# ajzhai/PEANUT

Measured on AMD Instinct MI355X. Metric: maps/sec for 480x480x(4+N_cat) prediction fwd, batch 32, higher is better.
Workload: dtype f32; 1 GPU; 480x480, 14-channel (4+10) partial maps -> 6-class prediction forward (PSPNet R50-V1c-D8), batch 32 per GPU, seeded random-init weights; survey_config=2, global_batch=32, parallelism=dp1 (map shards, no data-path collective)

## Files before the change

### peanut_amd/csrc/conv_pw_ares.hip

```cpp
#include <stdlib.h>

#include "common.h"
#include "conv_common.h"

namespace peanut {

namespace {

typedef const __attribute__((address_space(1))) void* gptr_t;
typedef __attribute__((address_space(3))) void* lptr_t;

__device__ __forceinline__ float load_uncounted(const float* ptr) {
  float v;
  asm volatile("global_load_dword %0, %1, off" : "=v"(v) : "v"(ptr) : "memory");
  return v;
}
template <int CH>
__device__ __forceinline__ void wait_uncounted(const float (&r)[CH], float a, float b) {
  static_assert(CH == 4 || CH == 8, "chunk of 4 or 8 values");
  __builtin_amdgcn_sched_barrier(0);
  if constexpr (CH == 4)
    asm volatile("s_waitcnt vmcnt(0)" ::"v"(r[0]), "v"(r[1]), "v"(r[2]), "v"(r[3]), "v"(a), "v"(b) : "memory");
  else
    asm volatile("s_waitcnt vmcnt(0)" ::"v"(r[0]), "v"(r[1]), "v"(r[2]), "v"(r[3]), "v"(r[4]), "v"(r[5]), "v"(r[6]), "v"(r[7]), "v"(a), "v"(b)
                 : "memory");
  __builtin_amdgcn_sched_barrier(0);
}

template <int NK, bool FLUSH>
__global__ __launch_bounds__(512) void conv_pw_ares_kernel(const ConvKParams p) {
  constexpr int BK = 32, K = NK * BK, TILE = 128 * BK;
  constexpr int CH = 32 / NK;
  static_assert(NK == 4 || NK == 8, "K = 128 or 256");
  __shared__ __attribute__((aligned(1024))) float smem[(NK + 2) * TILE];
  float* const bst = smem + NK * TILE;

  const int tid = threadIdx.x, lane = tid & 63;
  const int wave = __builtin_amdgcn_readfirstlane(tid >> 6);
  const int lr = lane >> 3, lp = lane & 7;
  const int wm = wave >> 2, wn = wave & 3;
  const int li = lane & 31, hi = lane >> 5;
  const bool late = p.phase_shift && wave >= 4;

  const int G = gridDim.x, bid = blockIdx.x;
  const int lw = (bid & 7) * (G >> 3) + (bid >> 3);
  const int NT = p.ntiles;
  const long long U = (long long)p.mtiles * NT;
  const int u0 = (int)(U * lw / G), u1 = (int)(U * (lw + 1) / G);
  if (u0 >= u1) return;

  const int pbn = p.ares_pbn;
  unsigned a_off[2], b_off[2];
#pragma unroll
  for (int j = 0; j < 2; ++j) {
    const int r = (wave * 2 + j) * 8 + lr;
    const int c = lp ^ ((r >> 1) & 7);
    a_off[j] = r * K + c * 4;
    b_off[j] = (r / pbn) * (NK * pbn * BK) + (r % pbn) * BK + c * 4;
  }
  auto dma_a = [&](int mt, int s) {
    const float* base = p.x + (size_t)mt * (128 * K) + s * BK;
#pragma unroll
    for (int j = 0; j < 2; ++j)
      __builtin_amdgcn_global_load_lds((gptr_t)(base + a_off[j]), (lptr_t)(smem + s * TILE + (wave * 2 + j) * 256), 16, 0, 0);
  };
  auto dma_b = [&](int mt, int nt, int kt, int stage) {
    const float* base = p.w + (p.mt_per_group ? (size_t)(mt / p.mt_per_group) * p.w_group_stride : 0) + (size_t)nt * (128 * K) + kt * (pbn * BK);
#pragma unroll
    for (int j = 0; j < 2; ++j)
      __builtin_amdgcn_global_load_lds((gptr_t)(base + b_off[j]), (lptr_t)(bst + stage * TILE + (wave * 2 + j) * 256), 16, 0, 0);
  };

  const int swz = (li >> 1) & 7;
  int sw[4];
#pragma unroll
  for (int ks = 0; ks < 4; ++ks) sw[ks] = ((ks * 2 + hi) ^ swz) * 4;
  const int a_row = (wm * 64 + li) * BK;
  const int b_row = (wn * 32 + li) * BK;

  f32x16 acc[2], acc2[2], prev[2];
#pragma unroll
  for (int t = 0; t < 2; ++t)
#pragma unroll
    for (int r = 0; r < 16; ++r) { acc[t][r] = 0.f; acc2[t][r] = 0.f; prev[t][r] = 0.f; }

  const size_t lane_el = (size_t)(wm * 64 + 4 * hi) * p.cout + wn * 32 + li;
  const bool has_res = p.res != nullptr;
  const size_t rstride = has_res ? (size_t)p.cout : 0;
  const size_t ostride = (size_t)p.cout;
  const float* res_run = has_res ? p.res + lane_el : p.zeros;
  float* out_run = p.y + lane_el;
  const float* prev_sc = p.scale + wn * 32 + li;
  const float* prev_sh = p.shift + wn * 32 + li;
  bool prev_valid = false;
  float scv = 1.f, shv = 0.f;
  const float alpha = p.alpha;
  const bool relu = p.relu != 0;

#define ARES_CHUNK_LOADS(kt)                                                              \
  float resv[CH];                                                                         \
  if ((kt) == 0) {                                                                        \
    scv = load_uncounted(prev_sc);                                                        \
    shv = load_uncounted(prev_sh);                                                        \
  }                                                                                       \
  _Pragma("unroll") for (int i = 0; i < CH; ++i)                                          \
    resv[i] = load_uncounted(res_run + (size_t)(8 * (i >> 2) + (i & 3)) * rstride);       \
  res_run += (size_t)(2 * CH) * rstride;
#define ARES_CHUNK_FINISH(kt)                                                             \
  if (prev_valid) {                                                   \
    _Pragma("unroll") for (int i = 0; i < CH; ++i) {                                      \
      const int idx = (kt) * CH + i;                                                      \
      float v = prev[idx >> 4][idx & 15] * (scv * alpha) + shv;                           \
      v += resv[i];                                                                       \
      if (relu) v = relu_keep_nan(v);                                                     \
      out_run[(size_t)(8 * (i >> 2) + (i & 3)) * ostride] = v;                            \
    }                                                                                     \
  }                                                                                       \
  out_run += (size_t)(2 * CH) * ostride;

  {
    const int mt = u0 / NT, nt = u0 - mt * NT;
#pragma unroll
    for (int s = 0; s < NK; ++s) dma_a(mt, s);
    dma_b(mt, nt, 0, 0);
    asm volatile("s_waitcnt vmcnt(0)" ::: "memory");
    __builtin_amdgcn_s_barrier();
    asm volatile("" ::: "memory");
  }

  int stage = 0;
  for (int u = u0; u < u1; ++u) {
    const int mt = u / NT, nt = u - mt * NT;
    const bool nxt = u + 1 < u1;
    const int mt_n = nxt ? (u + 1) / NT : mt;
    const int nt_n = nxt ? (u + 1) - mt_n * NT : 0;
    const bool refill_next = nxt && mt_n != mt;

    static_for<NK>([&](auto kc) {
      constexpr int kt = decltype(kc)::value;
      const float* const cur_b = bst + stage * TILE;
      const float* const cur_a = smem + kt * TILE;
      const bool more = (kt + 1 < NK) || nxt;
      ARES_CHUNK_LOADS(kt)
      auto request = [&]() {
        if (more) {
          if (kt + 1 < NK) dma_b(mt, nt, kt + 1, stage ^ 1);
          else dma_b(mt_n, nt_n, 0, stage ^ 1);
        }
      };
      if (!late) request();
      __builtin_amdgcn_sched_barrier(0);
      f32x4 af[4][2], bf[4];
#pragma unroll
      for (int j = 0; j < 4; ++j) {
        af[j][0] = *reinterpret_cast<const f32x4*>(cur_a + a_row + sw[j]);
        af[j][1] = *reinterpret_cast<const f32x4*>(cur_a + a_row + 32 * BK + sw[j]);
        bf[j] = *reinterpret_cast<const f32x4*>(cur_b + b_row + sw[j]);
      }
#pragma unroll
      for (int j = 0; j < 2; ++j)
#pragma unroll
        for (int kk = 0; kk < 4; ++kk)
#pragma unroll
          for (int t = 0; t < 2; ++t) acc[t] = __builtin_amdgcn_mfma_f32_32x32x2f32(af[j][t][kk], bf[j][kk], acc[t], 0, 0, 0);
      __builtin_amdgcn_sched_barrier(0);
      if (late) request();
      __builtin_amdgcn_sched_barrier(0);
#pragma unroll
      for (int j = 2; j < 4; ++j)
#pragma unroll
        for (int kk = 0; kk < 4; ++kk)
#pragma unroll
          for (int t = 0; t < 2; ++t) acc[t] = __builtin_amdgcn_mfma_f32_32x32x2f32(af[j][t][kk], bf[j][kk], acc[t], 0, 0, 0);
      if (FLUSH && (kt & 1)) {
#pragma unroll
        for (int t = 0; t < 2; ++t) {
          acc2[t] += acc[t];
#pragma unroll
          for (int r = 0; r < 16; ++r) acc[t][r] = 0.f;
        }
      }
      wait_uncounted<CH>(resv, scv, shv);
      ARES_CHUNK_FINISH(kt)
      if (kt >= 1) { if (refill_next) dma_a(mt_n, kt - 1); }
      asm volatile("s_waitcnt lgkmcnt(0)" ::: "memory");
      __builtin_amdgcn_s_barrier();
      asm volatile("" ::: "memory");
      stage ^= 1;
    });

#pragma unroll
    for (int t = 0; t < 2; ++t) {
      prev[t] = FLUSH ? acc2[t] : acc[t];
#pragma unroll
      for (int r = 0; r < 16; ++r) { acc[t][r] = 0.f; acc2[t][r] = 0.f; }
    }
    {
      const size_t unit_el = (size_t)mt * 128 * p.cout + (size_t)nt * 128 + lane_el;
      res_run = has_res ? p.res + unit_el : p.zeros;
      out_run = p.y + unit_el;
      const int ss_off = (p.mt_per_group && p.ss_group_stride) ? (mt / p.mt_per_group) * p.ss_group_stride : 0;
      prev_sc = p.scale + ss_off + nt * 128 + wn * 32 + li;
      prev_sh = p.shift + ss_off + nt * 128 + wn * 32 + li;
      prev_valid = true;
    }
    if (refill_next) dma_a(mt_n, NK - 1);
  }

  static_for<NK>([&](auto kc) {
    constexpr int kt = decltype(kc)::value;
    ARES_CHUNK_LOADS(kt)
    wait_uncounted<CH>(resv, scv, shv);
    ARES_CHUNK_FINISH(kt)
  });
#undef ARES_CHUNK_LOADS
#undef ARES_CHUNK_FINISH
}

template <int NK, bool FLUSH>
int launch_ares_t(ConvKParams p, hipStream_t stream) {
  int dev = 0, cus = 0;
  if (hipGetDevice(&dev) != hipSuccess || hipDeviceGetAttribute(&cus, hipDeviceAttributeMultiprocessorCount, dev) != hipSuccess || cus < 8)
    return fail(-3, "conv_pw_ares: no current device");
  const long long U = (long long)p.mtiles * p.ntiles;
  long long G = U < cus ? U : cus;
  G -= G % 8;
  if (G < 8) return fail(-2, "conv_pw_ares: launch too small");
  hipLaunchKernelGGL((conv_pw_ares_kernel<NK, FLUSH>), dim3((unsigned)G), dim3(512), 0, stream, p);
  hipError_t e = hipGetLastError();
  if (e != hipSuccess) return fail(-3, std::string("conv_pw_ares launch: ") + hipGetErrorString(e));
  return 0;
}

}

bool conv_pw_uses_ares(int cin, int cout, long long M, int stride, bool two_source, int flush_ktiles, int bn_tile) {
  const bool on = opt(OPT_PW_ARES) != 0;
  const long long min_units = opt(OPT_PW_ARES_MINUNITS);
  if (!on || two_source || (cin != 128 && cin != 256) || stride != 1 || M % 128 != 0 || cout % 128 != 0) return false;
  if (bn_tile != 64 && bn_tile != 128) return false;
  if (flush_ktiles != 0 && flush_ktiles != 2) return false;
  return (M / 128) * (cout / 128) >= min_units;
}

int launch_conv_pw_ares(const ConvKParams& p0, int bn_tile, hipStream_t stream) {
  ConvKParams p = p0;
  p.phase_shift = opt(OPT_PW256_PHASE) != 0;
  p.ares_pbn = bn_tile;
  p.mtiles = p.M / 128;
  p.ntiles = p.cout / 128;
  note_kernel("conv_pw_ares_128x128");
  const bool flush = p.flush == 2;
  if (p.c1 == 256) return flush ? launch_ares_t<8, true>(p, stream) : launch_ares_t<8, false>(p, stream);
  return flush ? launch_ares_t<4, true>(p, stream) : launch_ares_t<4, false>(p, stream);
}

}
```

### peanut_amd/csrc/options.h

```cpp
#pragma once
#include <stdlib.h>
#include <string.h>

#include <string>

namespace peanut {

enum OptionId {
  OPT_PW_GLDS, OPT_PW256_MINK, OPT_PW256_MINTILES, OPT_PW256_PHASE, OPT_PW256_SKIP_PAD, OPT_PW256W_MINK, OPT_PW256W_MINTILES, OPT_PW256P_MINK, OPT_PW256P_MINTILES, OPT_PW256P_FLUSH, OPT_PW256P_ORDER, OPT_PW256P_STREAMK, OPT_PW256WP_MINK, OPT_PW256WP_MINTILES, OPT_PW256WP_NPRE, OPT_PW256WP_STAGGER, OPT_PW_ARES, OPT_PW_SKINNY,
  OPT_PW_ARES_MINUNITS, OPT_PATCH_MINTILES, OPT_STEM_NCHW, OPT_BN64_MAXK, OPT_PW_BN64_MAXK, OPT_PW64_MAXTILES, OPT_FP32_BK, OPT_NCHUNK, OPT_RES_PREFETCH, OPT_SPLIT_MODEL,
  OPT_RS_CONV, OPT_RS_BN64_MAXK, OPT_RS256_MINK, OPT_RS256_MINTILES, OPT_RS64_MAXK, OPT_RS64_MAXTILES,
  OPT_WINO_M, OPT_WINO_HEAD_M, OPT_WINO6_MAXDIL, OPT_WINO5_MINDIL, OPT_WINO_FLUSH_CH, OPT_WINO_MIN_CIN, OPT_WINO_NARROW_MINPIX, OPT_WINO_SMALL_MAXWG, OPT_DEFER_SPLITK,
  OPT_PPM_OVERLAP, OPT_PPM_GROUPED, OPT_PPM_TERM_ROWS, OPT_PPM_GROUP_ROWS, OPT_RCNN_WINO_M, OPT_RCNN_STEM_S2D, OPT_RCNN_RPN_FUSED, OPT_RCNN_FPN_OVERLAP, OPT_RCNN_RANK_SORT, OPT_RCNN_TOPK_SLICE, OPT_RCNN_NMS_LEVELS, OPT_FMM_LOCAL32, OPT_FMM_MAX_PASSES, OPT_FMM_BLOCKED, OPT_FMM_INNER,
  OPT_COUNT
};

struct OptionInfo {
  const char* key;
  long long def;
  bool upload_time;
  const char* help;
};

inline const OptionInfo* option_table() {
  static const OptionInfo t[OPT_COUNT] = {
      {"pw_glds", 1, false, "fp32 1x1 convs / grouped GEMMs on the LDS-DMA kernels of conv_pw.hip (0: conv_igemm)"},
      {"pw256_mink", 1024, false, "fewest input channels for the 256 x 128 three-stage kernel"},
      {"pw256_mintiles", 256, false, "fewest 256 x 128 tiles for that kernel"},
      {"pw256_phase", 1, false, "the two waves of a SIMD request their LDS-DMA pieces half an iteration apart"},
      {"pw256_skip_pad", 1, false, "256 x 128 kernel, grouped GEMMs: waves whose rows are all group padding issue no MFMAs (0: compute the zero rows)"},
      {"pw256w_mink", 768, false, "fewest input channels for the 256 x 256 two-stage kernel (0: off)"},
      {"pw256w_mintiles", 1536, false, "fewest 256 x 256 tiles for that kernel"},
      {"pw256p_mink", 512, false, "fewest input channels for the persistent 256 x 128 kernel (conv_pw256p.hip; 0: off)"},
      {"pw256p_mintiles", 512, false, "fewest 256 x 128 tiles for that kernel"},
      {"pw256p_flush", 512, false, "most input channels of a Winograd position GEMM (two-level accumulation) that runs on the persistent kernel (0: none)"},
      {"pw256p_order", 1, false, "persistent 256 x 128 kernel: 1 = the workgroups of an XCD walk its run of tiles side by side (neighbours share operand panels in L2), 0 = one contiguous run per workgroup"},
      {"pw256p_streamk", 1, false, "persistent 256 x 128 kernel: the tail tiles' k-tiles as one stream in equal runs per workgroup (0: every tail tile cut into the same number of parts)"},
      {"pw256wp_mink", 512, false, "fewest input channels for the persistent 256 x 256 kernel (conv_pw256wp.hip; 0: off)"},
      {"pw256wp_mintiles", 768, false, "fewest 256 x 256 tiles for that kernel"},
      {"pw256wp_npre", 0, false, "persistent 256 x 256 kernel: accumulator blocks per in-place epilogue group (2 or 4; 0 = two with a residual, four without)"},
      {"pw256wp_stagger", 0, false, "persistent 256 x 256 kernel: spread of the workgroups' start times in sleeps of ~3.4 us (their tile boundaries -- 512 KiB of epilogue traffic per CU -- then fall at different times)"},
      {"pw_ares", 1, false, "K = 128 / 256 pointwise layers on the persistent A-resident kernel (conv_pw_ares.hip)"},
      {"pw_skinny", 1, false, "grouped pointwise launches with at most 64 data rows per group (the PSP pyramid's per-scale convs and Q tables at batch 1) on the skinny weight-streaming kernel (gemm_skinny.hip: 6 KiB of LDS, fits next to any other kernel; 0: the MFMA kernels on 128-row padded tiles)"},
      {"pw_ares_minunits", 512, false, "fewest (m-tile, n-tile) units for that kernel"},
      {"patch_mintiles", 1024, false, "3x3 convs of 16 / 32 input channels on the persistent LDS-patch kernel (conv_patch.hip) from this many 8 x 16 output tiles (0: off)"},
      {"stem_nchw", 1, false, "prediction forward: the first stem conv reads the NCHW input itself (conv_patch.hip, NCHW variant) instead of a layout pass + NHWC conv (fp32 mode, when the patch kernel takes the layer)"},
      {"bn64_maxk", 256, true, "128 x 64 tiles for layers with at most this many input channels"},
      {"pw_bn64_maxk", 128, true, "pointwise layers / Winograd position GEMMs: weights PACKED 64 wide up to this many input channels (wider layers: 128-wide packing, 64-wide tiles chosen per shape)"},
      {"pw64_maxtiles", 512, false, "a 128-wide-packed pointwise layer with at most bn64_maxk input channels runs 128 x 64 tiles while its 128 x 128 tiling has fewer tiles than this (two per CU)"},
      {"fp32_bk", 0, true, "16: force 16-channel k-tiles in conv_igemm (experiment)"},
      {"nchunk", 8, false, "n-tiles per chunk of the tile order (0: n fastest over all n-tiles)"},
      {"res_prefetch", 1, false, "request the first residual rows before the last k-tile's MFMAs"},
      {"split_model", 1, false, "tail split-K plan counts CUs (1) or resident slots (0)"},
      {"rs_conv", 1, true, "emulated modes: non-pointwise convs on conv_rs.hip (0: fp32 MFMA kernel)"},
      {"rs_bn64_maxk", 128, true, "emulated modes: 128 x 64 tiles up to this many input channels"},
      {"rs256_mink", 512, false, "emulated modes: fewest input channels for the 256 x 256 kernel"},
      {"rs256_mintiles", 256, false, "emulated modes: fewest 256 x 256 tiles for it"},
      {"rs64_maxk", 512, false, "emulated modes: 64 x 64 tiles up to this many input channels"},
      {"rs64_maxtiles", 128, false, "emulated modes: ... and below this many 128-row tiles"},
      {"wino_m", 0, true, "4 / 5 / 6: force one Winograd form on every eligible layer (0: policy)"},
      {"wino_head_m", 0, true, "4 / 5 / 6: Winograd form of the PSP bottleneck (0: policy)"},
      {"wino6_maxdil", 4, true, "largest dilation that gets an F(6x6) form"},
      {"wino5_mindil", 4, true, "smallest dilation that also gets an F(5x5) form (0: none)"},
      {"wino_flush_ch", 64, true, "channels per partial sum of the position GEMMs' two-level accumulation (0: off)"},
      {"wino_min_cin", 0, true, "fewest input channels of a Winograd layer (0: the planner's policy)"},
      {"wino_narrow_minpix", 20000, false, "layers under 128 channels take their Winograd form from this many input pixels on (round 6: 100 000 -> 20 000 -- with the small-problem transforms one 720 x 720 map's layer1 conv2, 32 400 pixels, gains 5 us per layer as F(6x6); profiles/r9e)"},
      {"wino_small_maxwg", 1024, false, "Winograd transforms: launches with fewer workgroups than this of the one-thread-per-tile kernels take the small-problem variants (a workgroup per tile and 64-channel slice, a thread per line, through LDS; bit-identical; 0: never)"},
      {"defer_splitk", 1, false, "a Bottleneck conv1 whose every tile is split along k leaves its partial tiles unsummed and conv2's (small-problem) Winograd input transform sums them: one launch fewer per block at batch 1, bit-identical (0: every conv runs its own reduce); read when a (B, H, W) plan is built"},
      {"ppm_overlap", -1, false, "pyramid branch of the PSP head on a side stream: 0 / 1, -1 = by size"},
      {"ppm_grouped", -1, false, "per-scale PSP GEMMs as one grouped launch: 0 / 1, -1 = by size"},
      {"ppm_term_rows", 1, false, "folded pyramid term: one wave per output row, no barrier in the row loop (0: the workgroup-wide two-phase kernel)"},
      {"ppm_group_rows", 0, false, "pyramid pooling, row pass: rows added up per workgroup (1..5; 0 = by size: as many as still leave ~768 workgroups)"},
      {"rcnn_wino_m", 0, true, "detector front end: 4 / 5 / 6 pins one Winograd form (0: per shape)"},
      {"rcnn_stem_s2d", 1, true, "detector stem 7x7 stride 2 as a space-to-depth 4x4 conv"},
      {"rcnn_rpn_fused", 1, false, "detector: the RPN head on all five pyramid levels as one chain (five input transforms, ONE grouped Winograd GEMM, five output transforms, one objectness and one anchor-delta GEMM over all levels' rows: 12 launches instead of 25); read when a (B, H, W) plan is built"},
      {"rcnn_fpn_overlap", 0, false, "detector: the FPN output convs of p5, p4, p3 on a side stream next to the lateral / top-down chain that ends in p2's (round 5 experiment, bit-identical; measured SLOWER at batch 1, 5.70 against 5.61 ms per frame, profiles/r8: off); read when a (B, H, W) plan is built"},
      {"rcnn_rank_sort", 1, false, "detector: the RPN candidates of an image are ordered by counting the larger keys (n / 64 workgroups) instead of one workgroup's bitonic sort (round 5; same order: the keys are distinct)"},
      {"rcnn_topk_slice", 20480, false, "detector: objectness logits per workgroup of the per-level top-k (a level is cut into up to 8 ranges whose k largest are merged by counting; 0: one workgroup per level, round 4)"},
      {"rcnn_nms_levels", 1, false, "detector: the proposal NMS level by level (five 16 x 16-word suppression blocks and five scans per image side by side, post-NMS top-k by counting) instead of one score-sorted list per image (round 5; same proposals)"},
      {"fmm_local32", 1, false, "goal solver: single-precision local solve inside a tile"},
      {"fmm_max_passes", 24, false, "goal solver: hard ceiling of the second-order ordering passes; they stop as soon as a pass changes nothing (6-10 passes on the agent's 960 x 960 map; peanut_goal_converged reports whether they reached their fixed point)"},
      {"fmm_blocked", 1, false, "goal solver: a wave relaxes its 8 x 8 block of the tile to convergence between workgroup barriers (round 5; 0: one Jacobi sweep of the whole tile per barrier pair)"},
      {"fmm_inner", 48, false, "goal solver: iterations a wave spends on its block before it publishes it (blocked rounds)"},
  };
  return t;
}

struct Options {
  long long v[OPT_COUNT];
};

inline int option_index(const char* key) {
  if (!key) return -1;
  std::string k(key);
  for (auto& c : k) c = (char)((c >= 'A' && c <= 'Z') ? c - 'A' + 'a' : c);
  if (k.rfind("peanut_", 0) == 0) k = k.substr(7);
  const OptionInfo* t = option_table();
  for (int i = 0; i < OPT_COUNT; ++i)
    if (k == t[i].key) return i;
  return -1;
}

inline Options& default_options() {
  static Options d = [] {
    Options o;
    const OptionInfo* t = option_table();
    for (int i = 0; i < OPT_COUNT; ++i) {
      o.v[i] = t[i].def;
      std::string env = "PEANUT_";
      for (const char* c = t[i].key; *c; ++c) env += (char)((*c >= 'a' && *c <= 'z') ? *c - 'a' + 'A' : *c);
      const char* e = getenv(env.c_str());
      if (e && *e) o.v[i] = atoll(e);
    }
    return o;
  }();
  return d;
}

inline const Options*& active_options_ptr() {
  static thread_local const Options* p = nullptr;
  return p;
}

inline long long opt(OptionId id) {
  const Options* a = active_options_ptr();
  return (a ? a : &default_options())->v[id];
}

struct OptionScope {
  const Options* saved;
  explicit OptionScope(const Options* o) : saved(active_options_ptr()) { active_options_ptr() = o; }
  ~OptionScope() { active_options_ptr() = saved; }
  OptionScope(const OptionScope&) = delete;
  OptionScope& operator=(const OptionScope&) = delete;
};

}
```

Before: 888.5 maps/s.

## Defer A-resident epilogue stores one iteration and keep them in flight

Adds a PIPE variant of the persistent A-resident pointwise kernel, enabled by default. Each chunk's epilogue values are computed into the prev registers and stored one k-iteration later, issued behind that iteration's loads. A counted vmcnt wait lets those stores stay in flight across the wait and barrier instead of draining every request. The A-panel refill also moves ahead of the residual loads. This targets the per-iteration stall on global store completion, at the cost of more code paths, extra variant macros and trace instrumentation, and reliance on exact vmcnt accounting.

```diff
diff --git a/peanut_amd/csrc/conv_pw_ares.hip b/peanut_amd/csrc/conv_pw_ares.hip
--- a/peanut_amd/csrc/conv_pw_ares.hip
+++ b/peanut_amd/csrc/conv_pw_ares.hip
@@ -27,7 +27,28 @@
   __builtin_amdgcn_sched_barrier(0);
 }
 
-template <int NK, bool FLUSH>
+template <int CH>
+__device__ __forceinline__ void wait_keep(const float (&r)[CH], float a, float b) {
+  static_assert(CH == 4 || CH == 8, "chunk of 4 or 8 values");
+  __builtin_amdgcn_sched_barrier(0);
+  if constexpr (CH == 4)
+    asm volatile("s_waitcnt vmcnt(4)" ::"v"(r[0]), "v"(r[1]), "v"(r[2]), "v"(r[3]), "v"(a), "v"(b) : "memory");
+  else
+    asm volatile("s_waitcnt vmcnt(8)" ::"v"(r[0]), "v"(r[1]), "v"(r[2]), "v"(r[3]), "v"(r[4]), "v"(r[5]), "v"(r[6]), "v"(r[7]), "v"(a), "v"(b)
+                 : "memory");
+  __builtin_amdgcn_sched_barrier(0);
+}
+
+#ifndef PEANUT_ARES_VARIANT
+#define PEANUT_ARES_VARIANT 0
+#endif
+#if PEANUT_ARES_VARIANT == 1
+#define ARES_PUT(ptr, v) asm volatile("" ::"v"(v))
+#else
+#define ARES_PUT(ptr, v) (*(ptr) = (v))
+#endif
+
+template <int NK, bool FLUSH, bool PIPE>
 __global__ __launch_bounds__(512) void conv_pw_ares_kernel(const ConvKParams p) {
   constexpr int BK = 32, K = NK * BK, TILE = 128 * BK;
   constexpr int CH = 32 / NK;
@@ -97,6 +118,11 @@
   const float alpha = p.alpha;
   const bool relu = p.relu != 0;
 
+#if PEANUT_ARES_VARIANT == 2
+#define ARES_CHUNK_LOADS(kt)                                                              \
+  float resv[CH];                                                                         \
+  _Pragma("unroll") for (int i = 0; i < CH; ++i) resv[i] = 0.f;
+#else
 #define ARES_CHUNK_LOADS(kt)                                                              \
   float resv[CH];                                                                         \
   if ((kt) == 0) {                                                                        \
@@ -106,30 +132,58 @@
   _Pragma("unroll") for (int i = 0; i < CH; ++i)                                          \
     resv[i] = load_uncounted(res_run + (size_t)(8 * (i >> 2) + (i & 3)) * rstride);       \
   res_run += (size_t)(2 * CH) * rstride;
+#endif
 #define ARES_CHUNK_FINISH(kt)                                                             \
-  if (prev_valid) {                                                   \
+  if (prev_valid) {                                                                       \
     _Pragma("unroll") for (int i = 0; i < CH; ++i) {                                      \
       const int idx = (kt) * CH + i;                                                      \
       float v = prev[idx >> 4][idx & 15] * (scv * alpha) + shv;                           \
       v += resv[i];                                                                       \
       if (relu) v = relu_keep_nan(v);                                                     \
-      out_run[(size_t)(8 * (i >> 2) + (i & 3)) * ostride] = v;                            \
+      ARES_PUT(out_run + (size_t)(8 * (i >> 2) + (i & 3)) * ostride, v);                  \
     }                                                                                     \
   }                                                                                       \
   out_run += (size_t)(2 * CH) * ostride;
+#define ARES_CHUNK_VALUES(kt)                                                             \
+  _Pragma("unroll") for (int i = 0; i < CH; ++i) {                                        \
+    const int idx = (kt) * CH + i;                                                        \
+    float v = prev[idx >> 4][idx & 15] * (scv * alpha) + shv;                             \
+    v += resv[i];                                                                         \
+    if (relu) v = relu_keep_nan(v);                                                       \
+    prev[idx >> 4][idx & 15] = v;                                                         \
+  }
+#define ARES_CHUNK_STORES(kt)                                                             \
+  _Pragma("unroll") for (int i = 0; i < CH; ++i) {                                        \
+    const int idx = (kt) * CH + i;                                                        \
+    ARES_PUT(out_run + (size_t)(8 * (i >> 2) + (i & 3)) * ostride, prev[idx >> 4][idx & 15]); \
+  }                                                                                       \
+  out_run += (size_t)(2 * CH) * ostride;
+
+#ifdef PEANUT_ARES_TRACE
+  unsigned long long tr_t0 = 0, tr_t1 = 0, tr_t2 = 0, tr_t3 = 0, tr_mfma = 0, tr_wait = 0, tr_tail = 0, tr_n = 0;
+#define ARES_STAMP(t)                                                                     \
+  __builtin_amdgcn_sched_barrier(0);                                                      \
+  asm volatile("s_memtime %0\n\ts_waitcnt lgkmcnt(0)" : "=s"(t)::"memory");               \
+  __builtin_amdgcn_sched_barrier(0);
+#endif
 
   {
     const int mt = u0 / NT, nt = u0 - mt * NT;
 #pragma unroll
     for (int s = 0; s < NK; ++s) dma_a(mt, s);
     dma_b(mt, nt, 0, 0);
+    if (PEANUT_ARES_VARIANT == 3) dma_b(mt, nt, 1, 1);
     asm volatile("s_waitcnt vmcnt(0)" ::: "memory");
     __builtin_amdgcn_s_barrier();
     asm volatile("" ::: "memory");
   }
+#ifdef PEANUT_ARES_TRACE
+  ARES_STAMP(tr_t0)
+#endif
 
   int stage = 0;
-  for (int u = u0; u < u1; ++u) {
+  auto run_unit = [&](int u, auto hp) {
+    constexpr bool HP = decltype(hp)::value != 0;
     const int mt = u / NT, nt = u - mt * NT;
     const bool nxt = u + 1 < u1;
     const int mt_n = nxt ? (u + 1) / NT : mt;
@@ -141,11 +195,20 @@
       const float* const cur_b = bst + stage * TILE;
       const float* const cur_a = smem + kt * TILE;
       const bool more = (kt + 1 < NK) || nxt;
+      constexpr bool ST = PIPE && HP && kt >= 1 && PEANUT_ARES_VARIANT != 1;
+      if constexpr (PIPE) {
+        if (kt >= 1) { if (refill_next) dma_a(mt_n, kt - 1); }
+      }
       ARES_CHUNK_LOADS(kt)
       auto request = [&]() {
-        if (more) {
+        if (more && PEANUT_ARES_VARIANT != 3) {
           if (kt + 1 < NK) dma_b(mt, nt, kt + 1, stage ^ 1);
           else dma_b(mt_n, nt_n, 0, stage ^ 1);
+        }
+        if constexpr (ST) {
+          __builtin_amdgcn_sched_barrier(0);
+          asm volatile("" ::: "memory");
+          ARES_CHUNK_STORES(kt - 1)
         }
       };
       if (!late) request();
@@ -180,12 +243,34 @@
           for (int r = 0; r < 16; ++r) acc[t][r] = 0.f;
         }
       }
-      wait_uncounted<CH>(resv, scv, shv);
-      ARES_CHUNK_FINISH(kt)
-      if (kt >= 1) { if (refill_next) dma_a(mt_n, kt - 1); }
+#ifdef PEANUT_ARES_TRACE
+      ARES_STAMP(tr_t1)
+#endif
+      if constexpr (PIPE) {
+        if constexpr (ST) wait_keep<CH>(resv, scv, shv);
+        else wait_uncounted<CH>(resv, scv, shv);
+#ifdef PEANUT_ARES_TRACE
+        ARES_STAMP(tr_t2)
+#endif
+        if constexpr (HP) {
+          ARES_CHUNK_VALUES(kt)
+          if constexpr (kt == NK - 1) { ARES_CHUNK_STORES(kt) }
+        }
+      } else {
+        wait_uncounted<CH>(resv, scv, shv);
+#ifdef PEANUT_ARES_TRACE
+        ARES_STAMP(tr_t2)
+#endif
+        ARES_CHUNK_FINISH(kt)
+        if (kt >= 1) { if (refill_next) dma_a(mt_n, kt - 1); }
+      }
       asm volatile("s_waitcnt lgkmcnt(0)" ::: "memory");
       __builtin_amdgcn_s_barrier();
       asm volatile("" ::: "memory");
+#ifdef PEANUT_ARES_TRACE
+      ARES_STAMP(tr_t3)
+      tr_mfma += tr_t1 - tr_t0; tr_wait += tr_t2 - tr_t1; tr_tail += tr_t3 - tr_t2; tr_t0 = tr_t3; ++tr_n;
+#endif
       stage ^= 1;
     });
 
@@ -205,6 +290,13 @@
       prev_valid = true;
     }
     if (refill_next) dma_a(mt_n, NK - 1);
+  };
+
+  if constexpr (PIPE) {
+    run_unit(u0, IC<0>{});
+    for (int u = u0 + 1; u < u1; ++u) run_unit(u, IC<1>{});
+  } else {
+    for (int u = u0; u < u1; ++u) run_unit(u, IC<0>{});
   }
 
   static_for<NK>([&](auto kc) {
@@ -213,11 +305,21 @@
     wait_uncounted<CH>(resv, scv, shv);
     ARES_CHUNK_FINISH(kt)
   });
+#ifdef PEANUT_ARES_TRACE
+  if (tid == 0) {
+    unsigned long long* const tr = reinterpret_cast<unsigned long long*>(p.partial) + bid * 4;
+    tr[0] = tr_mfma; tr[1] = tr_wait; tr[2] = tr_tail; tr[3] = tr_n;
+  }
+#undef ARES_STAMP
+#endif
 #undef ARES_CHUNK_LOADS
 #undef ARES_CHUNK_FINISH
-}
-
-template <int NK, bool FLUSH>
+#undef ARES_CHUNK_VALUES
+#undef ARES_CHUNK_STORES
+#undef ARES_PUT
+}
+
+template <int NK, bool FLUSH, bool PIPE>
 int launch_ares_t(ConvKParams p, hipStream_t stream) {
   int dev = 0, cus = 0;
   if (hipGetDevice(&dev) != hipSuccess || hipDeviceGetAttribute(&cus, hipDeviceAttributeMultiprocessorCount, dev) != hipSuccess || cus < 8)
@@ -226,10 +328,16 @@
   long long G = U < cus ? U : cus;
   G -= G % 8;
   if (G < 8) return fail(-2, "conv_pw_ares: launch too small");
-  hipLaunchKernelGGL((conv_pw_ares_kernel<NK, FLUSH>), dim3((unsigned)G), dim3(512), 0, stream, p);
+  hipLaunchKernelGGL((conv_pw_ares_kernel<NK, FLUSH, PIPE>), dim3((unsigned)G), dim3(512), 0, stream, p);
   hipError_t e = hipGetLastError();
   if (e != hipSuccess) return fail(-3, std::string("conv_pw_ares launch: ") + hipGetErrorString(e));
   return 0;
+}
+
+template <int NK>
+int launch_ares_nk(const ConvKParams& p, bool flush, bool pipe, hipStream_t stream) {
+  if (pipe) return flush ? launch_ares_t<NK, true, true>(p, stream) : launch_ares_t<NK, false, true>(p, stream);
+  return flush ? launch_ares_t<NK, true, false>(p, stream) : launch_ares_t<NK, false, false>(p, stream);
 }
 
 }
@@ -250,9 +358,9 @@
   p.mtiles = p.M / 128;
   p.ntiles = p.cout / 128;
   note_kernel("conv_pw_ares_128x128");
-  const bool flush = p.flush == 2;
-  if (p.c1 == 256) return flush ? launch_ares_t<8, true>(p, stream) : launch_ares_t<8, false>(p, stream);
-  return flush ? launch_ares_t<4, true>(p, stream) : launch_ares_t<4, false>(p, stream);
-}
-
-}
+  const bool flush = p.flush == 2, pipe = opt(OPT_PW_ARES_PIPE) != 0;
+  if (p.c1 == 256) return launch_ares_nk<8>(p, flush, pipe, stream);
+  return launch_ares_nk<4>(p, flush, pipe, stream);
+}
+
+}
diff --git a/peanut_amd/csrc/options.h b/peanut_amd/csrc/options.h
--- a/peanut_amd/csrc/options.h
+++ b/peanut_amd/csrc/options.h
@@ -8,7 +8,7 @@
 
 enum OptionId {
   OPT_PW_GLDS, OPT_PW256_MINK, OPT_PW256_MINTILES, OPT_PW256_PHASE, OPT_PW256_SKIP_PAD, OPT_PW256W_MINK, OPT_PW256W_MINTILES, OPT_PW256P_MINK, OPT_PW256P_MINTILES, OPT_PW256P_FLUSH, OPT_PW256P_ORDER, OPT_PW256P_STREAMK, OPT_PW256WP_MINK, OPT_PW256WP_MINTILES, OPT_PW256WP_NPRE, OPT_PW256WP_STAGGER, OPT_PW_ARES, OPT_PW_SKINNY,
-  OPT_PW_ARES_MINUNITS, OPT_PATCH_MINTILES, OPT_STEM_NCHW, OPT_BN64_MAXK, OPT_PW_BN64_MAXK, OPT_PW64_MAXTILES, OPT_FP32_BK, OPT_NCHUNK, OPT_RES_PREFETCH, OPT_SPLIT_MODEL,
+  OPT_PW_ARES_MINUNITS, OPT_PW_ARES_PIPE, OPT_PATCH_MINTILES, OPT_STEM_NCHW, OPT_BN64_MAXK, OPT_PW_BN64_MAXK, OPT_PW64_MAXTILES, OPT_FP32_BK, OPT_NCHUNK, OPT_RES_PREFETCH, OPT_SPLIT_MODEL,
   OPT_RS_CONV, OPT_RS_BN64_MAXK, OPT_RS256_MINK, OPT_RS256_MINTILES, OPT_RS64_MAXK, OPT_RS64_MAXTILES,
   OPT_WINO_M, OPT_WINO_HEAD_M, OPT_WINO6_MAXDIL, OPT_WINO5_MINDIL, OPT_WINO_FLUSH_CH, OPT_WINO_MIN_CIN, OPT_WINO_NARROW_MINPIX, OPT_WINO_SMALL_MAXWG, OPT_DEFER_SPLITK,
   OPT_PPM_OVERLAP, OPT_PPM_GROUPED, OPT_PPM_TERM_ROWS, OPT_PPM_GROUP_ROWS, OPT_RCNN_WINO_M, OPT_RCNN_STEM_S2D, OPT_RCNN_RPN_FUSED, OPT_RCNN_FPN_OVERLAP, OPT_RCNN_RANK_SORT, OPT_RCNN_TOPK_SLICE, OPT_RCNN_NMS_LEVELS, OPT_FMM_LOCAL32, OPT_FMM_MAX_PASSES, OPT_FMM_BLOCKED, OPT_FMM_INNER,
@@ -43,6 +43,7 @@
       {"pw_ares", 1, false, "K = 128 / 256 pointwise layers on the persistent A-resident kernel (conv_pw_ares.hip)"},
       {"pw_skinny", 1, false, "grouped pointwise launches with at most 64 data rows per group (the PSP pyramid's per-scale convs and Q tables at batch 1) on the skinny weight-streaming kernel (gemm_skinny.hip: 6 KiB of LDS, fits next to any other kernel; 0: the MFMA kernels on 128-row padded tiles)"},
       {"pw_ares_minunits", 512, false, "fewest (m-tile, n-tile) units for that kernel"},
+      {"pw_ares_pipe", 1, false, "A-resident kernel: a chunk's epilogue stores are issued one iteration late, behind that iteration's loads, and stay in flight across its wait and barrier (counted vmcnt; 0: every iteration waits for all its requests, the round-4 loop; bit-identical)"},
       {"patch_mintiles", 1024, false, "3x3 convs of 16 / 32 input channels on the persistent LDS-patch kernel (conv_patch.hip) from this many 8 x 16 output tiles (0: off)"},
       {"stem_nchw", 1, false, "prediction forward: the first stem conv reads the NCHW input itself (conv_patch.hip, NCHW variant) instead of a layout pass + NHWC conv (fp32 mode, when the patch kernel takes the layer)"},
       {"bn64_maxk", 256, true, "128 x 64 tiles for layers with at most this many input channels"},
```

Result: no change. 892.4 maps/s (median of 6 runs) (+0.4%).
